# thimabru1010/ResUnet-a_mltsk_keras

Hardware: AMD Instinct MI355X
Metric: training patches/sec (256×256, 6-ch, bs=8/GPU) at 1/2/4/8 MI355X (higher is better)
Workload: dtype bf16; 1 GPU; cfg3: ResUnet-a d6 multitask (seg+bound+dist+color) Tanimoto-dual, 256x256x6, 6 classes, Adam, full train step (fwd+loss+bwd+allreduce+update); global_batch=8, per_gpu_batch=8, parallelism=dp1

## Files before the change

### include/rua_hip.h

```cpp
#ifndef RUA_HIP_H
#define RUA_HIP_H
#include <stdint.h>
#ifdef __cplusplus
extern "C" {
#endif

#define RUA_F32 0
#define RUA_BF16 1
#define RUA_MAX_SEG 6
#define RUA_MAX_BRANCH 4
#define RUA_MAX_WGRAD_BATCH 32
#define RUA_MAX_WGRAD_GROUP 8

#define RUA_OK 0
#define RUA_ERR_ARG (-1)
#define RUA_ERR_LAUNCH (-2)

int rua_version(void);
const char* rua_last_error(void);
int rua_device_info(int* cu_count, int* lds_bytes, char* arch, int arch_len);

typedef struct rua_conv_seg {
  const void* x;
  const void* w;
// ... 215 lines not shown
int rua_pixel_loss(int kind, const float* p, const float* z, const float* y, const float* class_w,
                   int64_t M, int C, double* loss_out, float* per_pixel, void* stream);
int rua_head_dz(int kind, int act, const float* p, const float* y, const float* coef, const float* class_w,
                float grad_scale, int B, int64_t HW, int C, float* dz, void* stream);
int rua_seg_metrics(const float* p, const float* y, int64_t M, int C, double* out, void* stream);

int rua_lr_step(double* state, float* lr_out, int adam, double beta1, double beta2, void* stream);
int rua_adam_step(float* theta, float* g, float* m, float* v, int64_t n, float lr_t, const float* lr_t_dev, float beta1, float beta2,
                  float eps, float grad_scale, int zero_grad, void* stream);
int rua_sgd_step(float* theta, float* g, float* vel, int64_t n, float lr, const float* lr_dev, float momentum, float grad_scale,
                 int zero_grad, void* stream);
int rua_adam_step_w(float* theta, float* g, float* m, float* v, int64_t n, float lr_t, const float* lr_t_dev, float beta1, float beta2,
                    float eps, float grad_scale, int zero_grad, void* wcopy_bf16, void* stream);
int rua_sgd_step_w(float* theta, float* g, float* vel, int64_t n, float lr, const float* lr_dev, float momentum, float grad_scale,
                   int zero_grad, void* wcopy_bf16, void* stream);

int64_t rua_targets_scratch_bytes(int N, int num_classes);
int rua_multitask_targets(const uint8_t* img, const uint8_t* cls, int N, int H, int W, int Cin, int num_classes, int norm_type,
                          float* x, float* seg, float* bound, float* dist, float* color, void* scratch, int64_t scratch_bytes, void* stream);

int rua_scene_windows(const uint8_t* const* scene_img, const uint8_t* const* scene_cls, const int32_t* scene_h, const int32_t* scene_w,
                      int nscenes, const int32_t* windows, int N, int PH, int PW, int Cin,
                      uint8_t* img_out, uint8_t* cls_out, void* stream);

int rua_scene_windows_affine(const uint8_t* const* scene_img, const uint8_t* const* scene_cls, const int32_t* scene_h, const int32_t* scene_w,
                             int nscenes, const int32_t* windows , int N, int PH, int PW, int Cin,
                             uint8_t* img_out, uint8_t* cls_out, void* stream);

int rua_scene_stitch(const float* p, int N, int PH, int PW, int C, const int32_t* windows, const int32_t* own,
                     uint8_t* const* scene_pred, const uint8_t* const* scene_cls, const int32_t* scene_h, const int32_t* scene_w,
// ... 32 lines not shown
```

### resunet_a_mltsk_keras_amd/_lib.py

```python
from __future__ import annotations

import ctypes as C
import os

HERE = os.path.dirname(os.path.abspath(__file__))
LIB_PATH = os.environ.get("RUA_LIB_PATH") or os.path.join(HERE, "librua_hip.so")

RUA_F32, RUA_BF16 = 0, 1
RUA_MAX_SEG, RUA_MAX_BRANCH, RUA_MAX_WGRAD_GROUP, RUA_MAX_WGRAD_BATCH = 6, 4, 8, 32
LOSS_TANIMOTO, LOSS_WCE, LOSS_CE_LOGITS, LOSS_BCE_LOGITS, LOSS_MSE = 0, 1, 2, 3, 4
ACT_NONE, ACT_SOFTMAX, ACT_SIGMOID = 0, 1, 2

vp, i32, i64, f32, f64 = C.c_void_p, C.c_int32, C.c_int64, C.c_float, C.c_double


class ConvSeg(C.Structure):
    _fields_ = [("x", vp), ("w", vp), ("C", i32), ("Hs", i32), ("Ws", i32), ("up_shift", i32), ("dil", i32), ("taps", i32)]


class ConvDesc(C.Structure):
    _fields_ = [("seg", ConvSeg * RUA_MAX_SEG), ("nseg", i32), ("N", i32), ("H", i32), ("W", i32), ("Cout", i32),
                ("stride", i32), ("dtype", i32), ("bias", vp), ("aux", vp), ("aux_mode", i32), ("mscale", vp),
                ("mshift", vp), ("out_relu", i32), ("accumulate", i32), ("y", vp), ("out_stride", i32), ("OH", i32),
                ("OW", i32), ("stats", vp), ("stats_mode", i32), ("workspace", vp), ("workspace_bytes", i64), ("stats_replicas", i32),
# ... 36 lines not shown


class BnBwdBranch(C.Structure):
    _fields_ = [("g", vp), ("stats2", vp), ("replicas", i32), ("stats2_out", i32), ("gamma", vp), ("mean", vp), ("rstd", vp),
                ("scale", vp), ("shift", vp), ("dgamma", vp), ("dbeta", vp)]


class BnBwdDesc(C.Structure):
    _fields_ = [("x", vp), ("dskip", vp), ("dx", vp), ("M", i64), ("C", i32), ("dtype", i32), ("nb", i32), ("masked", i32),
                ("accumulate", i32), ("pad", i32), ("count", f64), ("br", BnBwdBranch * RUA_MAX_BRANCH),
                ("skip_stats", vp), ("skip_replicas", i32), ("pad2", i32), ("dx_stats", vp), ("dx_replicas", i32), ("pad3", i32)]


class WprepItem(C.Structure):
    _fields_ = [("src_off", i64), ("dst_off", i64), ("taps", i32), ("Cout", i32), ("C", i32), ("pad", i32)]


PP = C.POINTER(vp)

_SIGS = {
    "rua_version": ([], i32),
    "rua_device_info": ([C.POINTER(i32), C.POINTER(i32), C.c_char_p, i32], i32),
    "rua_conv_fwd": ([C.POINTER(ConvDesc), vp], i32),
    "rua_conv_fwd_group": ([C.POINTER(ConvDesc), i32, vp], i32),
    "rua_conv_smem_bytes": ([C.POINTER(ConvDesc)], i32),
    "rua_conv_tile_bn": ([C.POINTER(ConvDesc)], i32),
    "rua_conv_tile_bm": ([C.POINTER(ConvDesc)], i32),
    "rua_conv_kernel_id": ([C.POINTER(ConvDesc)], i32),
    "rua_conv_fused_input_ok": ([C.POINTER(ConvDesc)], i32),
    "rua_conv_last_ksplit": ([], i32),
# ... 63 lines not shown
    "rua_fill_zero": ([vp, i64, vp], i32),
    "rua_tanimoto_sums": ([vp, vp, i32, i64, i32, vp, vp], i32),
    "rua_tanimoto_finalize": ([vp, i32, i64, i32, f32, vp, vp, vp, vp], i32),
    "rua_tanimoto_finalize_rep": ([vp, i32, i32, i64, i32, f32, vp, vp, vp, vp], i32),
    "rua_tanimoto_finalize_multi": ([vp, i32, vp], i32),
    "rua_head_dz_multi": ([vp, i32, vp], i32),
    "rua_tanimoto_ratio": ([vp, i32, i32, vp, vp, vp], i32),
    "rua_pixel_loss": ([i32, vp, vp, vp, vp, i64, i32, vp, vp, vp], i32),
    "rua_head_dz": ([i32, i32, vp, vp, vp, vp, f32, i32, i64, i32, vp, vp], i32),
    "rua_seg_metrics": ([vp, vp, i64, i32, vp, vp], i32),
    "rua_lr_step": ([vp, vp, i32, f64, f64, vp], i32),
    "rua_adam_step": ([vp, vp, vp, vp, i64, f32, vp, f32, f32, f32, f32, i32, vp], i32),
    "rua_sgd_step": ([vp, vp, vp, i64, f32, vp, f32, f32, i32, vp], i32),
    "rua_adam_step_w": ([vp, vp, vp, vp, i64, f32, vp, f32, f32, f32, f32, i32, vp, vp], i32),
    "rua_sgd_step_w": ([vp, vp, vp, i64, f32, vp, f32, f32, i32, vp, vp], i32),
    "rua_targets_scratch_bytes": ([i32, i32], i64),
    "rua_multitask_targets": ([vp, vp, i32, i32, i32, i32, i32, i32, vp, vp, vp, vp, vp, vp, i64, vp], i32),
    "rua_scene_windows": ([vp, vp, vp, vp, i32, vp, i32, i32, i32, i32, vp, vp, vp], i32),
    "rua_scene_windows_affine": ([vp, vp, vp, vp, i32, vp, i32, i32, i32, i32, vp, vp, vp], i32),
    "rua_scene_stitch": ([vp, i32, i32, i32, i32, vp, vp, vp, vp, vp, vp, i32, vp, vp], i32),
    "rua_scene_stitch_views": ([vp, i32, i32, i32, i32, i32, vp, vp, vp, vp, vp, vp, i32, vp, vp], i32),
    "rua_scene_stitch_maps": ([vp, i32, i32, i32, i32, i32, vp, vp, vp, vp, vp, i32, i32, vp], i32),
    "rua_scene_class_counts": ([vp, vp, vp, i32, vp, i32, i32, i32, i32, vp, vp], i32),
    "rua_scene_erode": ([vp, vp, vp, i32, i32, vp, vp, i32, vp, vp], i32),
    "rua_scene_boundary": ([vp, vp, vp, vp, i32, i32, i32, vp, vp, vp, vp], i32),
    "rua_set_tuning": ([C.c_char_p, i64], i32),
    "rua_get_tuning": ([C.c_char_p, C.POINTER(i64)], i32),
    "rua_tuning_key": ([i32], C.c_char_p),
}

# ... 66 lines not shown
```

### resunet_a_mltsk_keras_amd/build.py

```python
import os
import subprocess
import sys

HERE = os.path.dirname(os.path.abspath(__file__))
CSRC = os.path.join(HERE, "csrc")
OUT = os.environ.get("RUA_BUILD_OUT") or os.path.join(HERE, "librua_hip.so")
SOURCES = ["conv_mfma.hip", "conv_strip.hip", "conv_band.hip", "conv_band64.hip", "conv_band128.hip", "conv_img2.hip", "elementwise.hip", "small_conv.hip", "loss_optim.hip", "targets.hip", "scene.hip", "capi.cpp"]
FILE_FLAGS = {"conv_strip.hip": ["-fno-slp-vectorize"]}


def needs_build():
    if not os.path.exists(OUT):
        return True
    t = os.path.getmtime(OUT)
    deps = [os.path.join(CSRC, f) for f in os.listdir(CSRC)] + [os.path.join(HERE, "..", "include", "rua_hip.h")]
    return any(os.path.getmtime(d) > t for d in deps)


def build(force=False, verbose=True):
    if not force and not needs_build():
        return OUT
    hipcc = os.environ.get("HIPCC", "/opt/rocm/bin/hipcc")
    if not os.path.exists(hipcc):
        raise RuntimeError(f"hipcc not found at {hipcc}")
# ... 23 lines not shown
```

### resunet_a_mltsk_keras_amd/csrc/conv_mfma.hip

```cpp
#include "common.h"


template <typename T> __device__ __forceinline__ void load8(const unsigned char* base, size_t elem_off, float* f) {
  if constexpr (sizeof(T) == 2) {
    ET<T>::unpack(ldg16(base + elem_off * 2), f);
  } else {
    ET<T>::unpack(ldg16(base + elem_off * 4), f);
    ET<T>::unpack(ldg16(base + elem_off * 4 + 16), f + 4);
  }
}
template <typename T> __device__ __forceinline__ void store8(unsigned char* base, size_t elem_off, const float* f) {
  if constexpr (sizeof(T) == 2) {
    stg16(base + elem_off * 2, ET<T>::pack(f));
  } else {
    stg16(base + elem_off * 4, ET<T>::pack(f));
    stg16(base + elem_off * 4 + 16, ET<T>::pack(f + 4));
  }
}

template <typename T, int BM, int BN> __host__ __device__ constexpr int conv_smem_base() {
  constexpr int ROWB = (sizeof(T) == 2) ? 80 : 132;
  constexpr int a = 2 * (BM + BN) * ROWB;
  constexpr int b = BM * (BN + 4) * 4 + 4 * (BN / 8) * 16 * 4;
  return ((a > b ? a : b) + 15) / 16 * 16;
// ... 2295 lines not shown
}
struct WgKB { WgK k[RUA_MAX_WGRAD_BATCH]; unsigned end[RUA_MAX_WGRAD_BATCH]; int n; };
static_assert(sizeof(WgKB) <= 4096, "batched launch: kernel arguments are limited to 4 KiB");
__global__ __launch_bounds__(256) void wgrad_kernel_b(const WgKB g) {
  const unsigned b = blockIdx.x;
  int m = 0;
  for (int i = 0; i + 1 < g.n; ++i) m += (b >= g.end[i]) ? 1 : 0;
  const unsigned first = m ? g.end[m - 1] : 0u;
  wgrad_kernel_body<bf16_t>(g.k[m], (int)(b - first));
}

constexpr int SLAB_RED_COLS = 256;
__device__ __forceinline__ void wgrad_slab_reduce_body(const float* __restrict__ slabs, float* __restrict__ dw, long long n4, int ksplit, int vblock, int overwrite = 0) {
  const long long i = (long long)vblock * SLAB_RED_COLS + threadIdx.x;
  if (i >= n4) return;
  const float4* s = reinterpret_cast<const float4*>(slabs) + i;
  float4 t = make_float4(0.f, 0.f, 0.f, 0.f);
  auto add4 = [](float4& a, const float4 b) { a.x += b.x; a.y += b.y; a.z += b.z; a.w += b.w; };
  int k = 0;
  for (; k + 8 <= ksplit; k += 8) {
    float4 v[8];
#pragma unroll
    for (int u = 0; u < 8; ++u) v[u] = s[(size_t)(k + u) * n4];
    float4 a = v[0], b = v[4];
    add4(a, v[1]); add4(b, v[5]); add4(a, v[2]); add4(b, v[6]); add4(a, v[3]); add4(b, v[7]);
    add4(a, b); add4(t, a);
  }
  for (; k < ksplit; ++k) add4(t, s[(size_t)k * n4]);
  float4* d = reinterpret_cast<float4*>(dw) + i;
  float4 o = make_float4(0.f, 0.f, 0.f, 0.f);
  if (!overwrite) o = *d;
  add4(o, t);
  *d = o;
}
__global__ __launch_bounds__(256) void wgrad_slab_reduce(const float* __restrict__ slabs, float* __restrict__ dw, long long n4, int ksplit) {
  wgrad_slab_reduce_body(slabs, dw, n4, ksplit, (int)blockIdx.x);
}
static int launch_slab_reduce(const float* slabs, float* dw, long long n, int ksplit, hipStream_t st) {
  const long long n4 = n / 4;
  hipLaunchKernelGGL(wgrad_slab_reduce, dim3((unsigned)((n4 + SLAB_RED_COLS - 1) / SLAB_RED_COLS)), dim3(256), 0, st, slabs, dw, n4, ksplit);
  RUA_LAUNCH_CHECK("wgrad_slab_reduce");
  return RUA_OK;
}
static int slab_capacity(const rua_wgrad_desc* d, long long ndw);

struct WgdK {
  const unsigned char* a; const unsigned char* dy; float* dw;
  int C, Cout, H, W, dil, taps, wsh;
// ... 1199 lines not shown
#pragma unroll
    for (int q = 1; q < 4; ++q) v += *reinterpret_cast<const f32x4*>(src + q * 9 * 16 * 64);
    float* dst = p.dw + ((size_t)tap * p.Cout + co0 + col) * p.C + ci0 + c4;
    if (!ow) v += *reinterpret_cast<const f32x4*>(dst);
    *reinterpret_cast<f32x4*>(dst) = v;
  }
}

constexpr int TAPS_RED_COLS = 64;
__device__ __forceinline__ void wgrad_taps_reduce_body(const float* __restrict__ scratch, float* __restrict__ dw, int CC, int gx, int vblock, int overwrite = 0) {
  __shared__ float4 sh[256];
  const int total4 = 9 * CC * CC / 4;
  const int el = threadIdx.x & 63, sl = threadIdx.x >> 6;
  const int e4 = vblock * TAPS_RED_COLS + el;
  float4 s = make_float4(0.f, 0.f, 0.f, 0.f);
  auto add4 = [](float4& a, const float4 b) { a.x += b.x; a.y += b.y; a.z += b.z; a.w += b.w; };
  if (e4 < total4) {
    const int e = e4 * 4;
    const int tap = e / (CC * CC), r = e - tap * CC * CC, co = r / CC, ci = r - co * CC;
    const float* src = scratch + ((size_t)(co >> 5) * gx * 9 + tap) * 32 * CC + (co & 31) * CC + ci;
    const size_t pstride = (size_t)9 * 32 * CC;
    int b = sl;
    for (; b + 28 < gx; b += 32) {
      float4 v[8];
#pragma unroll
      for (int u = 0; u < 8; ++u) v[u] = *reinterpret_cast<const float4*>(src + (size_t)(b + 4 * u) * pstride);
      float4 a = v[0], c = v[4];
      add4(a, v[1]); add4(c, v[5]); add4(a, v[2]); add4(c, v[6]); add4(a, v[3]); add4(c, v[7]);
      add4(a, c); add4(s, a);
    }
    for (; b < gx; b += 4) add4(s, *reinterpret_cast<const float4*>(src + (size_t)b * pstride));
  }
  sh[threadIdx.x] = s;
  __syncthreads();
  if (sl == 0 && e4 < total4) {
    float4 t = sh[el];
    add4(t, sh[64 + el]); add4(t, sh[128 + el]); add4(t, sh[192 + el]);
    float4* d = reinterpret_cast<float4*>(dw + (size_t)e4 * 4);
    float4 o = make_float4(0.f, 0.f, 0.f, 0.f);
    if (!overwrite) o = *d;
    add4(o, t);
    *d = o;
  }
}

__global__ __launch_bounds__(256) void wgrad_taps_reduce(const float* __restrict__ scratch, float* __restrict__ dw, int CC, int gx) {
  wgrad_taps_reduce_body(scratch, dw, CC, gx, (int)blockIdx.x);
}

struct WgGroupCapture {
  int n;
  int kind[RUA_MAX_WGRAD_GROUP];
  unsigned gx[RUA_MAX_WGRAD_GROUP]; int smem[RUA_MAX_WGRAD_GROUP];
  WgK g[RUA_MAX_WGRAD_GROUP]; WgdK d[RUA_MAX_WGRAD_GROUP]; WgtK t[RUA_MAX_WGRAD_GROUP];
  int post[RUA_MAX_WGRAD_GROUP];
  const float* part[RUA_MAX_WGRAD_GROUP]; float* dw[RUA_MAX_WGRAD_GROUP]; long long ndw[RUA_MAX_WGRAD_GROUP]; int parts[RUA_MAX_WGRAD_GROUP], CC[RUA_MAX_WGRAD_GROUP], rblocks[RUA_MAX_WGRAD_GROUP];
};
// ... 1164 lines not shown
```

### resunet_a_mltsk_keras_amd/engine.py

```python
from __future__ import annotations

import ctypes as C
import math
import os
from dataclasses import dataclass, field
from typing import Dict, List, Optional, Tuple

import numpy as np
import torch

from . import _lib as L
from .scenes import MAP_HEADS, AffineSceneBatch, SceneBatch, check_radius, check_tolerance, check_views, view_rows

BN_EPS, BN_MOMENTUM, KERAS_EPS = 1e-3, 0.99, 1e-7
HEADS = ["seg", "bound", "dist", "color"]
SUMS_REPLICAS = 1


@dataclass
class ModelConfig:
    input_shape: Tuple[int, int, int] = (256, 256, 3)
    num_classes: int = 5
    multitasking: bool = False
    variant: str = "model2"
    width: int = 32
    depth: int = 6
# ... 249 lines not shown
        self.B = batch
        self.training = training
        self.dev = eng.dev
        self.dt = eng.dt
        self.tdt = torch.bfloat16 if eng.dt == L.RUA_BF16 else torch.float32
        self.vec = 8 if eng.dt == L.RUA_BF16 else 4
        self.fwd = Plan(dry)
        self.bwd = Plan(dry)
        self.loss_plan = Plan(dry)
        self.back_steps: List = _BackSteps(self)
        self.cur_tag: Optional[str] = None
        self.block_tag = ""
        self.pending: List[tuple] = []
        self.pending_bytes = 0
        self.pending_bucket = 0
        self.later: List[tuple] = []
        self.allocs: List[torch.Tensor] = []
        self.stats_used = 16
        self.act_bytes = 0
        self.img_u8 = self.cls_u8 = self.tgt_scratch = None
        self._build()

    def compact_buffers(self):
        if self.img_u8 is None:
            H, W, Cin = self.cfg.input_shape
            self.img_u8 = torch.empty((self.B, H, W, Cin), dtype=torch.uint8, device=self.dev)
            self.cls_u8 = torch.empty((self.B, H, W), dtype=torch.uint8, device=self.dev)
            n = int(L.lib().raw("rua_targets_scratch_bytes")(self.B, self.cfg.num_classes))
            self.tgt_scratch = torch.empty((max(n, 4),), dtype=torch.uint8, device=self.dev)
        return self.img_u8, self.cls_u8, self.tgt_scratch
# ... 408 lines not shown
        self.pending_bytes += nbytes

    def flush_wgrad(self, plan: Plan):
        self._issue_later(plan)
        self.pending_bytes = 0
        if not self.pending:
            return
        blocks = 0
        for r, _ in self.pending:
            r.block_begin = blocks
            blocks += r.blocks
        recs = (L.WgradPending * len(self.pending))(*[r for r, _ in self.pending])
        table = torch.frombuffer(bytearray(bytes(recs)), dtype=torch.uint8).to(self.dev)
        self.allocs.append(table)
        plan.add("rua_wgrad_reduce_batch", table.data_ptr(), len(self.pending), blocks, grads=[off for _, off in self.pending])
        self.pending = []

    def bias_grad(self, plan: Plan, dy: Ten, bias_offs: List[int]):
        s = self.col_stats(plan, dy)
        self.stats_to_grads(plan, s, dy.C, bias_offs)

    def stats_to_grads(self, plan: Plan, s: Stat, Cc: int, offs: List[int]):
        if self.dry or not (self.e.defer_reduce and plan is self.bwd):
            dst = L.ptr_array([self.G(o) for o in offs])
            plan.keep.append(dst)
            plan.add("rua_stats_to_f32", s.ptr, s.R, Cc, dst, len(offs), grads=offs)
            return
        for o in offs:
            bucket = self.e.dist.bucket_of(o) if self.e.dist is not None else 0
            if (self.pending or self.later) and bucket != self.pending_bucket:
                self.flush_wgrad(plan)
# ... 789 lines not shown
            raise L.RuaError("no HIP device visible: the ResUnet-a training path runs on MI355X only (there is no CPU fallback)")
        self.dev = device or torch.device("cuda", torch.cuda.current_device())
        cu = C.c_int32(0)
        if L.lib().raw("rua_device_info")(C.byref(cu), None, None, 0) == 0 and cu.value > 0:
            self.cu_count = cu.value
        z = lambda n, dt=torch.float32: torch.zeros(max(n, 16), dtype=dt, device=self.dev)
        self.P, self.G, self.M1, self.V1, self.S = z(ps.n), z(ps.n + ps.ns + 16), z(ps.n), z(ps.n), z(ps.ns)
        tdt = torch.bfloat16 if dtype == "bf16" else torch.float32
        self.Wf, self.Wd = z(ps.n, tdt), z(ps.n, tdt)
        self.wgrad_overwrite = os.environ.get("RUA_WGRAD_OVERWRITE", "1") != "0"
        self.ow_flag = torch.zeros(4, dtype=torch.int32, device=self.dev)
        self._ow = 0
        self._g_pending = False
        self.opt_wcopy = dtype == "bf16" and os.environ.get("RUA_OPT_WCOPY", "1") != "0"
        self.wf_fresh = False
        items = np.zeros(0, dtype=[("src", "<i8"), ("dst", "<i8"), ("taps", "<i4"), ("cout", "<i4"), ("c", "<i4"), ("pad", "<i4")])
        rows, mx = [], 1
        for lay in self.layers:
            if "segs" in lay and lay["mfma"]:
                for sg in lay["segs"]:
                    rows.append((sg["off"], sg["dst"], lay["taps"], lay["cout"], sg["C"], 0))
                    mx = max(mx, lay["taps"] * lay["cout"] * sg["C"])
        items = np.array(rows, dtype=items.dtype)
        self.wprep_items = torch.from_numpy(np.frombuffer(items.tobytes(), dtype=np.uint8).copy()).to(self.dev)
        self.wprep_n, self.wprep_max = len(rows), mx
        bm = []
        for i, (_, _, taps, cout, ci, _) in enumerate(rows):
            for b in range(L.lib().raw("rua_wprep_blocks")(taps, cout, ci)):
                bm += [i, 8 * b]
        self.wprep_map = torch.tensor(bm if bm else [0, 0], dtype=torch.int32, device=self.dev)
        self.wprep_map_n = len(bm) // 2
        self.stats_arena = torch.zeros(1 << 22, dtype=torch.float64, device=self.dev)
        self.workspace = torch.zeros(8 << 20, dtype=torch.float32, device=self.dev)
        self.scratch = torch.zeros(32 << 20, dtype=torch.float32, device=self.dev)
        self.lr_dev = torch.zeros(16, dtype=torch.float32, device=self.dev)
        self.lr_state = torch.zeros(2, dtype=torch.float64, device=self.dev)
        self._t_dev, self._lr_base_dev = -1, None
        self._dp_fence = torch.zeros(16, dtype=torch.float32, device=self.dev)
        self.use_graph = os.environ.get("RUA_USE_GRAPH", "1") != "0"
        self.group_1x1 = os.environ.get("RUA_GROUP_1X1", "1") != "0"
        self.group_heads = os.environ.get("RUA_GROUP_HEADS", "1") != "0"
        self.multi_head = os.environ.get("RUA_MULTI_HEAD", "1") != "0"
        self.merge_wgrad = {int(v) for v in os.environ.get("RUA_MERGE_WGRAD", "1,32,64,128,256").split(",") if v}
        self.group_wgrad_pw = os.environ.get("RUA_GROUP_WGRAD_PW", "1") != "0"
        self.batch_wgrad = os.environ.get("RUA_BATCH_WGRAD", "1") != "0"
        self.stem_mfma = os.environ.get("RUA_STEM_MFMA", "1") != "0"
# ... 57 lines not shown
        self._eval_seen = set()
        self._opt_graph = None
        self.graphs = {}
        cu = C.c_int32(0)
        if self.dev is not None and L.lib().raw("rua_device_info")(C.byref(cu), None, None, 0) == 0 and cu.value > 0:
            self.cu_count = cu.value

    def set_weights(self, keras_dict: Dict[str, np.ndarray]):
        P, S = self.params.from_keras(keras_dict)
        self.P.copy_(torch.from_numpy(P)); self.S.copy_(torch.from_numpy(S))
        self.params_changed()

    def params_changed(self):
        self.weights_dirty = True
        self.wf_fresh = False

    def get_weights(self) -> Dict[str, np.ndarray]:
        return self.params.to_keras(self.P.cpu().numpy(), self.S.cpu().numpy())

    def grads_keras(self) -> Dict[str, np.ndarray]:
        return self.params.to_keras(self.G.cpu().numpy())

    def count_params(self) -> int:
        return self.params.count()

    def _stream(self) -> int:
        return torch.cuda.current_stream(self.dev).cuda_stream

    def _prep_weights(self, s):
        if self.weights_dirty:
            if self.opt_wcopy and self.wf_fresh:
                L.lib().call("rua_weight_prep_dgrad", self.Wf.data_ptr(), self.Wd.data_ptr(), self.wprep_items.data_ptr(), self.wprep_n, self.wprep_max,
                             self.wprep_map.data_ptr() if self.wprep_map_n else None, self.wprep_map_n, self.dt, C.c_void_p(s))
            else:
                L.lib().call("rua_weight_prep", self.P.data_ptr(), self.Wf.data_ptr(), self.Wd.data_ptr(), self.wprep_items.data_ptr(),
                             self.wprep_n, self.wprep_max, self.dt, C.c_void_p(s))
                self.wf_fresh = True
            self.weights_dirty = False

    def _ensure_forward_copy(self):
        if self.opt_wcopy and not self.wf_fresh:
            self.weights_dirty = True
            self._prep_weights(self._stream())

    def _upload(self, g: Graph, x, y):
        def put(dst: torch.Tensor, src):
            if src is None:
                return
            if isinstance(src, np.ndarray):
                src = torch.from_numpy(np.ascontiguousarray(src, dtype=np.float32))
            if tuple(src.shape) != tuple(dst.shape):
                raise ValueError(f"expected shape {tuple(dst.shape)}, got {tuple(src.shape)}")
            dst.copy_(src, non_blocking=bool(src.is_pinned()) if isinstance(src, torch.Tensor) else False)
        put(g.x_in.t, x)
        if y is not None:
            if isinstance(y, dict):
# ... 129 lines not shown

    def _bucket_hooks(self, g: Graph):
        if getattr(g, "_hooks", None) is None:
            red = self.dist.reducer
            g._hooks = {idx: (lambda bs=bs: [red.ready(b) for b in bs]) for idx, bs in self._bucket_marks(g).items()}
        return g._hooks

    def _set_lr(self):
        sp = self.loss
        if self._t_dev != self.t or self._lr_base_dev != sp.lr:
            self.lr_state.copy_(torch.tensor([float(self.t), float(sp.lr)], dtype=torch.float64))
            self._t_dev, self._lr_base_dev = self.t, sp.lr
        self.t += 1
        self._t_dev += 1

    def _launch_optimizer(self, grad_scale, s):
        sp = self.loss
        L.lib().call("rua_lr_step", self.lr_state.data_ptr(), self.lr_dev.data_ptr(), 1 if sp.optimizer == "adam" else 0,
                     float(sp.beta_1), float(sp.beta_2), C.c_void_p(s))
        wc = self.Wf.data_ptr() if self.opt_wcopy else None
        if sp.optimizer == "adam":
            L.lib().call("rua_adam_step_w", self.P.data_ptr(), self.G.data_ptr(), self.M1.data_ptr(), self.V1.data_ptr(), self.params.n,
                         0.0, self.lr_dev.data_ptr(), sp.beta_1, sp.beta_2, KERAS_EPS, grad_scale, 1, wc, C.c_void_p(s))
        else:
            L.lib().call("rua_sgd_step_w", self.P.data_ptr(), self.G.data_ptr(), self.M1.data_ptr(), self.params.n, 0.0,
                         self.lr_dev.data_ptr(), sp.momentum, grad_scale, 1, wc, C.c_void_p(s))

    def optimizer_step(self, grad_scale: float = 1.0):
        self._set_lr()
        self._launch_optimizer(grad_scale, self._stream())
        self.weights_dirty = True
        self._g_pending = False

    def _issue_step(self, g: Graph):
        s = self._stream()
        self._zero_arena(g, s)
        self.weights_dirty = True
        self._prep_weights(s)
        g.fwd.run(s)
        g.loss_plan.run(s)
        g.bwd.run(s)
        self._launch_optimizer(1.0, s)

    def _graph_step(self, x, y, norm_type: Optional[int] = None):
        B = x.shape[0] if x is not None else self._last_B
        self._last_B = B
        g = self.graph(B, True)
        self._put_batch(g, x, y, norm_type)
        self._set_lr()
        self._set_overwrite(1 if (self.wgrad_overwrite and not self._g_pending) else 0)
        self._g_pending = False
        cap = self._captured.get(B)
        if cap is None:
            self._issue_step(g)
            torch.cuda.synchronize()
            cap = torch.cuda.CUDAGraph()
            with torch.cuda.graph(cap):
                self._issue_step(g)
            self._captured[B] = cap
            self.weights_dirty = True
            return g
        self._ensure_forward_copy()
        cap.replay()
        self.weights_dirty = True
        return g

    def count_step_dispatches(self, batch: int) -> Optional[int]:
        try:
            g = self.graph(batch, True)
            torch.cuda.synchronize()
            cap = torch.cuda.CUDAGraph(keep_graph=True)
            dirty, fresh = self.weights_dirty, self.wf_fresh
            with torch.cuda.graph(cap):
                self._issue_step(g)
            self.weights_dirty, self.wf_fresh = dirty, fresh
            k = C.c_int32(0)
            L.lib().call("rua_graph_kernel_nodes", C.c_void_p(cap.raw_cuda_graph()), C.byref(k), None)
            del cap
            return int(k.value)
        except Exception:
            torch.cuda.synchronize()
            return None

    def _graph_step_dp(self, x, y, norm_type: Optional[int] = None):
        B = x.shape[0] if x is not None else self._last_B
        self._last_B = B
        g = self.graph(B, True)
        self._put_batch(g, x, y, norm_type)
        red = self.dist.reducer
        pieces = self._captured_dp.get(B)
# ... 215 lines not shown
```

Before: 1343 patches/s.

## Fuse final wgrad reduction, optimizer update and bf16 weight-copy prep into one kernel

```diff
diff --git a/include/rua_hip.h b/include/rua_hip.h
--- a/include/rua_hip.h
+++ b/include/rua_hip.h
@@ -253,6 +253,19 @@
                     float eps, float grad_scale, int zero_grad, void* wcopy_bf16, void* stream);
 int rua_sgd_step_w(float* theta, float* g, float* vel, int64_t n, float lr, const float* lr_dev, float momentum, float grad_scale,
                    int zero_grad, void* wcopy_bf16, void* stream);
+typedef struct rua_optim_fused {
+  int32_t optimizer, pad;
+  float* theta; float* g; float* m; float* v;
+  int64_t n;
+  float lr; const float* lr_dev;
+  float beta1, beta2, eps, momentum, grad_scale, pad2;
+  void* w_fwd; void* w_dgrad;
+  const rua_wprep_item* items; int32_t n_items, n_pending;
+  const int32_t* item_rec;
+  const rua_wgrad_pending* pending;
+  const int32_t* blockmap; int32_t n_blocks, pad3;
+} rua_optim_fused;
+int rua_optim_step_fused(const rua_optim_fused* d, void* stream);
 
 int64_t rua_targets_scratch_bytes(int N, int num_classes);
 int rua_multitask_targets(const uint8_t* img, const uint8_t* cls, int N, int H, int W, int Cin, int num_classes, int norm_type,
diff --git a/resunet_a_mltsk_keras_amd/_lib.py b/resunet_a_mltsk_keras_amd/_lib.py
--- a/resunet_a_mltsk_keras_amd/_lib.py
+++ b/resunet_a_mltsk_keras_amd/_lib.py
@@ -74,6 +74,12 @@
 
 class WprepItem(C.Structure):
     _fields_ = [("src_off", i64), ("dst_off", i64), ("taps", i32), ("Cout", i32), ("C", i32), ("pad", i32)]
+
+
+class OptimFused(C.Structure):
+    _fields_ = [("optimizer", i32), ("pad", i32), ("theta", vp), ("g", vp), ("m", vp), ("v", vp), ("n", i64), ("lr", f32), ("lr_dev", vp),
+                ("beta1", f32), ("beta2", f32), ("eps", f32), ("momentum", f32), ("grad_scale", f32), ("pad2", f32), ("w_fwd", vp), ("w_dgrad", vp),
+                ("items", vp), ("n_items", i32), ("n_pending", i32), ("item_rec", vp), ("pending", vp), ("blockmap", vp), ("n_blocks", i32), ("pad3", i32)]
 
 
 PP = C.POINTER(vp)
@@ -167,6 +173,7 @@
     "rua_sgd_step": ([vp, vp, vp, i64, f32, vp, f32, f32, i32, vp], i32),
     "rua_adam_step_w": ([vp, vp, vp, vp, i64, f32, vp, f32, f32, f32, f32, i32, vp, vp], i32),
     "rua_sgd_step_w": ([vp, vp, vp, i64, f32, vp, f32, f32, i32, vp, vp], i32),
+    "rua_optim_step_fused": ([C.POINTER(OptimFused), vp], i32),
     "rua_targets_scratch_bytes": ([i32, i32], i64),
     "rua_multitask_targets": ([vp, vp, i32, i32, i32, i32, i32, i32, vp, vp, vp, vp, vp, vp, i64, vp], i32),
     "rua_scene_windows": ([vp, vp, vp, vp, i32, vp, i32, i32, i32, i32, vp, vp, vp], i32),
diff --git a/resunet_a_mltsk_keras_amd/build.py b/resunet_a_mltsk_keras_amd/build.py
--- a/resunet_a_mltsk_keras_amd/build.py
+++ b/resunet_a_mltsk_keras_amd/build.py
@@ -5,7 +5,7 @@
 HERE = os.path.dirname(os.path.abspath(__file__))
 CSRC = os.path.join(HERE, "csrc")
 OUT = os.environ.get("RUA_BUILD_OUT") or os.path.join(HERE, "librua_hip.so")
-SOURCES = ["conv_mfma.hip", "conv_strip.hip", "conv_band.hip", "conv_band64.hip", "conv_band128.hip", "conv_img2.hip", "elementwise.hip", "small_conv.hip", "loss_optim.hip", "targets.hip", "scene.hip", "capi.cpp"]
+SOURCES = ["conv_mfma.hip", "conv_strip.hip", "conv_band.hip", "conv_band64.hip", "conv_band128.hip", "conv_img2.hip", "elementwise.hip", "small_conv.hip", "loss_optim.hip", "optim_fused.hip", "targets.hip", "scene.hip", "capi.cpp"]
 FILE_FLAGS = {"conv_strip.hip": ["-fno-slp-vectorize"]}
 
 
diff --git a/resunet_a_mltsk_keras_amd/csrc/conv_mfma.hip b/resunet_a_mltsk_keras_amd/csrc/conv_mfma.hip
--- a/resunet_a_mltsk_keras_amd/csrc/conv_mfma.hip
+++ b/resunet_a_mltsk_keras_amd/csrc/conv_mfma.hip
@@ -1,4 +1,5 @@
 #include "common.h"
+#include "wgrad_reduce.h"
 
 
 template <typename T> __device__ __forceinline__ void load8(const unsigned char* base, size_t elem_off, float* f) {
@@ -2333,24 +2334,11 @@
 __device__ __forceinline__ void wgrad_slab_reduce_body(const float* __restrict__ slabs, float* __restrict__ dw, long long n4, int ksplit, int vblock, int overwrite = 0) {
   const long long i = (long long)vblock * SLAB_RED_COLS + threadIdx.x;
   if (i >= n4) return;
-  const float4* s = reinterpret_cast<const float4*>(slabs) + i;
-  float4 t = make_float4(0.f, 0.f, 0.f, 0.f);
-  auto add4 = [](float4& a, const float4 b) { a.x += b.x; a.y += b.y; a.z += b.z; a.w += b.w; };
-  int k = 0;
-  for (; k + 8 <= ksplit; k += 8) {
-    float4 v[8];
-#pragma unroll
-    for (int u = 0; u < 8; ++u) v[u] = s[(size_t)(k + u) * n4];
-    float4 a = v[0], b = v[4];
-    add4(a, v[1]); add4(b, v[5]); add4(a, v[2]); add4(b, v[6]); add4(a, v[3]); add4(b, v[7]);
-    add4(a, b); add4(t, a);
-  }
-  for (; k < ksplit; ++k) add4(t, s[(size_t)k * n4]);
+  const float4 t = wgrad_slab_sum(reinterpret_cast<const float4*>(slabs) + i, (size_t)n4, ksplit);
   float4* d = reinterpret_cast<float4*>(dw) + i;
   float4 o = make_float4(0.f, 0.f, 0.f, 0.f);
   if (!overwrite) o = *d;
-  add4(o, t);
-  *d = o;
+  *d = wgrad_finish(o, t);
 }
 __global__ __launch_bounds__(256) void wgrad_slab_reduce(const float* __restrict__ slabs, float* __restrict__ dw, long long n4, int ksplit) {
   wgrad_slab_reduce_body(slabs, dw, n4, ksplit, (int)blockIdx.x);
@@ -3580,33 +3568,15 @@
   const int el = threadIdx.x & 63, sl = threadIdx.x >> 6;
   const int e4 = vblock * TAPS_RED_COLS + el;
   float4 s = make_float4(0.f, 0.f, 0.f, 0.f);
-  auto add4 = [](float4& a, const float4 b) { a.x += b.x; a.y += b.y; a.z += b.z; a.w += b.w; };
-  if (e4 < total4) {
-    const int e = e4 * 4;
-    const int tap = e / (CC * CC), r = e - tap * CC * CC, co = r / CC, ci = r - co * CC;
-    const float* src = scratch + ((size_t)(co >> 5) * gx * 9 + tap) * 32 * CC + (co & 31) * CC + ci;
-    const size_t pstride = (size_t)9 * 32 * CC;
-    int b = sl;
-    for (; b + 28 < gx; b += 32) {
-      float4 v[8];
-#pragma unroll
-      for (int u = 0; u < 8; ++u) v[u] = *reinterpret_cast<const float4*>(src + (size_t)(b + 4 * u) * pstride);
-      float4 a = v[0], c = v[4];
-      add4(a, v[1]); add4(c, v[5]); add4(a, v[2]); add4(c, v[6]); add4(a, v[3]); add4(c, v[7]);
-      add4(a, c); add4(s, a);
-    }
-    for (; b < gx; b += 4) add4(s, *reinterpret_cast<const float4*>(src + (size_t)b * pstride));
-  }
+  if (e4 < total4) s = wgrad_taps_lane_sum(wgrad_taps_src(scratch, CC, gx, e4 * 4), wgrad_taps_pstride(CC), gx, sl);
   sh[threadIdx.x] = s;
   __syncthreads();
   if (sl == 0 && e4 < total4) {
-    float4 t = sh[el];
-    add4(t, sh[64 + el]); add4(t, sh[128 + el]); add4(t, sh[192 + el]);
+    const float4 t = wgrad_taps_fold(sh[el], sh[64 + el], sh[128 + el], sh[192 + el]);
     float4* d = reinterpret_cast<float4*>(dw + (size_t)e4 * 4);
     float4 o = make_float4(0.f, 0.f, 0.f, 0.f);
     if (!overwrite) o = *d;
-    add4(o, t);
-    *d = o;
+    *d = wgrad_finish(o, t);
   }
 }
 
diff --git a/resunet_a_mltsk_keras_amd/csrc/optim_fused.hip b/resunet_a_mltsk_keras_amd/csrc/optim_fused.hip
--- /dev/null
+++ b/resunet_a_mltsk_keras_amd/csrc/optim_fused.hip
@@ -0,0 +1,236 @@
+#include "common.h"
+#include "wgrad_reduce.h"
+
+struct AdamUpd {
+  static constexpr bool HAS_V = true;
+  float lr, b1, b2, eps, gs;
+  template <bool TAIL>
+  __device__ __forceinline__ void apply(float gg_, float& mm, float& vv, float& tt) const {
+#pragma clang fp contract(off)
+    const float gg = gg_ * gs, a1 = 1.f - b1, a2 = 1.f - b2;
+    if constexpr (TAIL) { mm = __builtin_fmaf(b1, mm, a1 * gg); vv = __builtin_fmaf(b2, vv, (a2 * gg) * gg); }
+    else { mm = __builtin_fmaf(a1, gg, b1 * mm); vv = __builtin_fmaf(gg, a2 * gg, b2 * vv); }
+    const float q = (lr * mm) / (sqrtf(vv) + eps);
+    tt = tt - q;
+  }
+};
+struct SgdUpd {
+  static constexpr bool HAS_V = false;
+  float lr, mu, gs;
+  template <bool TAIL>
+  __device__ __forceinline__ void apply(float gg, float& vel, float&, float& tt) const {
+#pragma clang fp contract(off)
+    const float vv = __builtin_fmaf(mu, vel, -((lr * gg) * gs));
+    vel = vv;
+    tt = tt + vv;
+  }
+};
+
+struct OptK {
+  float* th; float* g; float* m; float* v;
+  unsigned short* wf; unsigned short* wd;
+  const rua_wprep_item* items; const int* item_rec; const rua_wgrad_pending* pend; const int4* blockmap; const float* lr_dev;
+  long long ntail;
+};
+
+__device__ __forceinline__ float4 ld4(const float* p) { return *reinterpret_cast<const float4*>(p); }
+__device__ __forceinline__ void st4(float* p, const float4 v) { *reinterpret_cast<float4*>(p) = v; }
+
+template <typename U>
+__device__ __forceinline__ uint2 update4(const OptK& k, const U& u, size_t i, const float4 g4) {
+  float4 m4 = ld4(k.m + i), t4 = ld4(k.th + i), v4 = make_float4(0.f, 0.f, 0.f, 0.f);
+  if constexpr (U::HAS_V) v4 = ld4(k.v + i);
+  u.template apply<false>(g4.x, m4.x, v4.x, t4.x); u.template apply<false>(g4.y, m4.y, v4.y, t4.y); u.template apply<false>(g4.z, m4.z, v4.z, t4.z); u.template apply<false>(g4.w, m4.w, v4.w, t4.w);
+  st4(k.m + i, m4); st4(k.th + i, t4);
+  if constexpr (U::HAS_V) st4(k.v + i, v4);
+  return make_uint2(ET<bf16_t>::pk(t4.x, t4.y), ET<bf16_t>::pk(t4.z, t4.w));
+}
+template <typename U>
+__device__ __forceinline__ unsigned short update1(const OptK& k, const U& u, size_t i, float gg) {
+  float mm = k.m[i], tt = k.th[i], vv = 0.f;
+  if constexpr (U::HAS_V) vv = k.v[i];
+  if ((long long)i >= k.ntail) u.template apply<true>(gg, mm, vv, tt); else u.template apply<false>(gg, mm, vv, tt);
+  k.m[i] = mm; k.th[i] = tt;
+  if constexpr (U::HAS_V) k.v[i] = vv;
+  return __builtin_bit_cast(unsigned short, (bf16_t)tt);
+}
+
+template <int RK>
+__device__ __forceinline__ float4 grad4(float* __restrict__ garena, const float* __restrict__ part, int parts, int CC, size_t n_item, int e, bool ow) {
+  const float4 zero = make_float4(0.f, 0.f, 0.f, 0.f);
+  if constexpr (RK == 0) {
+    const float4 g4 = ld4(garena + e);
+    st4(garena + e, zero);
+    return g4;
+  } else {
+    float4 t;
+    if constexpr (RK == 1) {
+      const float* src = wgrad_taps_src(part, CC, parts, e);
+      const size_t ps = wgrad_taps_pstride(CC);
+      const float4 s0 = wgrad_taps_lane_sum(src, ps, parts, 0); __builtin_amdgcn_sched_barrier(0);
+      const float4 s1 = wgrad_taps_lane_sum(src, ps, parts, 1); __builtin_amdgcn_sched_barrier(0);
+      const float4 s2 = wgrad_taps_lane_sum(src, ps, parts, 2); __builtin_amdgcn_sched_barrier(0);
+      const float4 s3 = wgrad_taps_lane_sum(src, ps, parts, 3); __builtin_amdgcn_sched_barrier(0);
+      t = wgrad_taps_fold(s0, s1, s2, s3);
+    } else {
+      t = wgrad_slab_sum(reinterpret_cast<const float4*>(part + e), n_item / 4, parts);
+    }
+    float4 o = zero;
+    if (!ow) { o = ld4(garena + e); st4(garena + e, zero); }
+    return wgrad_finish(o, t);
+  }
+}
+
+template <typename U, int RK>
+__device__ __forceinline__ void tile_rows(const OptK& k, const U& u, const rua_wprep_item& it, int t, int tco, int tci, const float* part, int parts, int CC, bool ow) {
+  const int lane = threadIdx.x & 63, cg = lane >> 3, pg = lane & 7;
+  const int tap = t / (tco * tci), r = t - tap * tco * tci;
+  const int co = (r / tci) * 64 + cg * 8, ci = (r % tci) * 64 + pg * 8;
+  if (co >= it.Cout || ci >= it.C) return;
+  const size_t n_item = (size_t)it.taps * it.Cout * it.C;
+  uint4 in[8];
+#pragma unroll
+  for (int q = 0; q < 8; ++q) in[q] = make_uint4(0u, 0u, 0u, 0u);
+#pragma nounroll
+  for (int j = 0; j < 8; ++j) {
+    const int e = (tap * it.Cout + co + j) * it.C + ci;
+    const float4 g0 = grad4<RK>(k.g + it.src_off, part, parts, CC, n_item, e, ow);
+    if constexpr (RK != 0) __builtin_amdgcn_sched_barrier(0);
+    const float4 g1 = grad4<RK>(k.g + it.src_off, part, parts, CC, n_item, e + 4, ow);
+    const uint2 lo = update4(k, u, (size_t)it.src_off + e, g0), hi = update4(k, u, (size_t)it.src_off + e + 4, g1);
+    const uint4 pk = make_uint4(lo.x, lo.y, hi.x, hi.y);
+    *reinterpret_cast<uint4*>(k.wf + it.dst_off + e) = pk;
+#pragma unroll
+    for (int q = 0; q < 8; ++q) if (q == j) in[q] = pk;
+  }
+  unsigned short* dp = k.wd + it.dst_off + (size_t)(it.taps - 1 - tap) * it.Cout * it.C + (size_t)ci * it.Cout + co;
+#pragma unroll
+  for (int i = 0; i < 8; ++i) {
+    unsigned e[8];
+#pragma unroll
+    for (int j = 0; j < 8; ++j) {
+      const unsigned w = (i >> 1) == 0 ? in[j].x : (i >> 1) == 1 ? in[j].y : (i >> 1) == 2 ? in[j].z : in[j].w;
+      e[j] = (i & 1) ? (w >> 16) : (w & 0xffffu);
+    }
+    *reinterpret_cast<uint4*>(dp + (size_t)i * it.Cout) = make_uint4(e[0] | (e[1] << 16), e[2] | (e[3] << 16), e[4] | (e[5] << 16), e[6] | (e[7] << 16));
+  }
+}
+
+template <typename U>
+__global__ __launch_bounds__(256) void optim_fused_kernel(const OptK k, U u) {
+  __shared__ unsigned short tile[64][66];
+  if (k.lr_dev) u.lr = k.lr_dev[0];
+  const int4 bm = k.blockmap[blockIdx.x];
+  const int tid = threadIdx.x;
+  if (bm.x == 0) {
+#pragma unroll
+    for (int q = 0; q < 4; ++q) {
+      const int c = q * 256 + tid;
+      if (c < bm.w) {
+        const size_t i = ((size_t)bm.z + c) * 4;
+        const float4 g4 = ld4(k.g + i);
+        st4(k.g + i, make_float4(0.f, 0.f, 0.f, 0.f));
+        *reinterpret_cast<uint2*>(k.wf + i) = update4(k, u, i, g4);
+      }
+    }
+    return;
+  }
+  if (bm.x == 3) {
+    if (tid < bm.w) {
+      const size_t i = (size_t)bm.z + tid;
+      const float gg = k.g[i];
+      k.g[i] = 0.f;
+      k.wf[i] = update1(k, u, i, gg);
+    }
+    return;
+  }
+  const rua_wprep_item it = k.items[bm.y];
+  const int rec = k.item_rec ? k.item_rec[bm.y] : -1;
+  int rk = 0, parts = 0, CC = 0; const float* part = nullptr; bool ow = false;
+  if (rec >= 0) {
+    const rua_wgrad_pending p = k.pend[rec];
+    rk = p.kind; parts = p.parts; CC = p.CC; part = p.partials;
+    ow = p.overwrite_dev && *p.overwrite_dev != 0;
+  }
+  const int tco = (it.Cout + 63) / 64, tci = (it.C + 63) / 64;
+  if (bm.x == 1) {
+    const int wv = tid >> 6;
+    for (int t = bm.z + wv; t < bm.z + bm.w; t += 4) {
+      if (rk == 1) tile_rows<U, 1>(k, u, it, t, tco, tci, part, parts, CC, ow);
+      else if (rk == 2) tile_rows<U, 2>(k, u, it, t, tco, tci, part, parts, CC, ow);
+      else tile_rows<U, 0>(k, u, it, t, tco, tci, part, parts, CC, ow);
+    }
+    return;
+  }
+  const int tx = tid & 15, ty = tid >> 4;
+  const size_t n_item = (size_t)it.taps * it.Cout * it.C;
+  const bool vec = (it.C % 4 == 0) && (it.Cout % 4 == 0);
+  for (int t = bm.z; t < bm.z + bm.w; ++t) {
+    const int tap = t / (tco * tci), r = t - tap * tco * tci;
+    const int co0 = (r / tci) * 64, ci0 = (r % tci) * 64;
+#pragma nounroll
+    for (int q = 0; q < 4; ++q) {
+      const int co = co0 + ty + q * 16;
+#pragma nounroll
+      for (int j = 0; j < 4; ++j) {
+        const int ci = ci0 + tx * 4 + j;
+        unsigned short b = 0;
+        if (co < it.Cout && ci < it.C) {
+          const size_t e = (size_t)tap * it.Cout * it.C + (size_t)co * it.C + ci, i = (size_t)it.src_off + e;
+          float gg;
+          if (rk == 2) {
+            const float s = wgrad_slab_sum(part + e, n_item, parts);
+            float o = 0.f;
+            if (!ow) { o = k.g[i]; k.g[i] = 0.f; }
+            gg = wgrad_finish(o, s);
+          } else { gg = k.g[i]; k.g[i] = 0.f; }
+          b = update1(k, u, i, gg);
+          k.wf[it.dst_off + e] = b;
+        }
+        tile[ty + q * 16][tx * 4 + j] = b;
+      }
+    }
+    __syncthreads();
+#pragma unroll
+    for (int q = 0; q < 4; ++q) {
+      const int ci = ci0 + ty + q * 16, co = co0 + tx * 4;
+      if (ci < it.C) {
+        unsigned short v[4];
+#pragma unroll
+        for (int j = 0; j < 4; ++j) v[j] = tile[tx * 4 + j][ty + q * 16];
+        unsigned short* d = k.wd + it.dst_off + (size_t)(it.taps - 1 - tap) * it.Cout * it.C + (size_t)ci * it.Cout + co;
+        if (vec && co + 3 < it.Cout) *reinterpret_cast<uint2*>(d) = make_uint2((unsigned)v[0] | ((unsigned)v[1] << 16), (unsigned)v[2] | ((unsigned)v[3] << 16));
+        else {
+#pragma unroll
+          for (int j = 0; j < 4; ++j) if (co + j < it.Cout) d[j] = v[j];
+        }
+      }
+    }
+    __syncthreads();
+  }
+}
+
+extern "C" int rua_optim_step_fused(const rua_optim_fused* d, void* stream) {
+  RUA_CHECK_ARG(d, "rua_optim_step_fused: null descriptor");
+  RUA_CHECK_ARG(d->theta && d->g && d->m && (d->v || d->optimizer == 1) && d->n > 0 && d->n < ((int64_t)1 << 31), "rua_optim_step_fused: bad buffers");
+  RUA_CHECK_ARG(d->optimizer == 0 || d->optimizer == 1, "rua_optim_step_fused: optimizer must be 0 (Adam) or 1 (SGD)");
+  RUA_CHECK_ARG(d->w_fwd && d->w_dgrad && d->w_fwd != d->w_dgrad, "rua_optim_step_fused: needs both bf16 weight copies");
+  RUA_CHECK_ARG((((size_t)d->theta | (size_t)d->g | (size_t)d->m | (size_t)d->v | (size_t)d->w_fwd | (size_t)d->w_dgrad) & 15) == 0, "rua_optim_step_fused: buffers must be 16-byte aligned");
+  RUA_CHECK_ARG(d->blockmap && d->n_blocks >= 1 && ((size_t)d->blockmap & 15) == 0, "rua_optim_step_fused: needs a block map (16-byte aligned)");
+  RUA_CHECK_ARG(d->n_items >= 0 && (d->n_items == 0 || d->items), "rua_optim_step_fused: bad item table");
+  RUA_CHECK_ARG(d->n_pending >= 0 && (d->n_pending == 0 || (d->pending && d->item_rec)), "rua_optim_step_fused: pending records need their table and the items' record indices");
+  OptK k;
+  k.th = d->theta; k.g = d->g; k.m = d->m; k.v = d->v;
+  k.wf = (unsigned short*)d->w_fwd; k.wd = (unsigned short*)d->w_dgrad;
+  k.items = d->items; k.item_rec = d->n_pending > 0 ? d->item_rec : nullptr; k.pend = d->pending;
+  k.blockmap = (const int4*)d->blockmap; k.lr_dev = d->lr_dev; k.ntail = d->n & ~(int64_t)3;
+  if (d->optimizer == 0) {
+    const AdamUpd u{d->lr, d->beta1, d->beta2, d->eps, d->grad_scale};
+    hipLaunchKernelGGL((optim_fused_kernel<AdamUpd>), dim3(d->n_blocks), dim3(256), 0, (hipStream_t)stream, k, u);
+  } else {
+    const SgdUpd u{d->lr, d->momentum, d->grad_scale};
+    hipLaunchKernelGGL((optim_fused_kernel<SgdUpd>), dim3(d->n_blocks), dim3(256), 0, (hipStream_t)stream, k, u);
+  }
+  RUA_LAUNCH_CHECK("rua_optim_step_fused");
+  return RUA_OK;
+}
diff --git a/resunet_a_mltsk_keras_amd/csrc/wgrad_reduce.h b/resunet_a_mltsk_keras_amd/csrc/wgrad_reduce.h
--- /dev/null
+++ b/resunet_a_mltsk_keras_amd/csrc/wgrad_reduce.h
@@ -0,0 +1,50 @@
+#pragma once
+#include <hip/hip_runtime.h>
+
+__device__ __forceinline__ void rua_acc(float4& a, const float4 b) { a.x += b.x; a.y += b.y; a.z += b.z; a.w += b.w; }
+__device__ __forceinline__ void rua_acc(float& a, const float b) { a += b; }
+template <typename V> __device__ __forceinline__ V rua_vzero();
+template <> __device__ __forceinline__ float4 rua_vzero<float4>() { return make_float4(0.f, 0.f, 0.f, 0.f); }
+template <> __device__ __forceinline__ float rua_vzero<float>() { return 0.f; }
+
+template <typename V>
+__device__ __forceinline__ V wgrad_slab_sum(const V* __restrict__ s, size_t stride, int ksplit) {
+  V t = rua_vzero<V>();
+  int k = 0;
+  for (; k + 8 <= ksplit; k += 8) {
+    V v[8];
+#pragma unroll
+    for (int u = 0; u < 8; ++u) v[u] = s[(size_t)(k + u) * stride];
+    V a = v[0], b = v[4];
+    rua_acc(a, v[1]); rua_acc(b, v[5]); rua_acc(a, v[2]); rua_acc(b, v[6]); rua_acc(a, v[3]); rua_acc(b, v[7]);
+    rua_acc(a, b); rua_acc(t, a);
+  }
+  for (; k < ksplit; ++k) rua_acc(t, s[(size_t)k * stride]);
+  return t;
+}
+
+__device__ __forceinline__ size_t wgrad_taps_pstride(int CC) { return (size_t)9 * 32 * CC; }
+__device__ __forceinline__ const float* wgrad_taps_src(const float* __restrict__ scratch, int CC, int gx, int e) {
+  const int tap = e / (CC * CC), r = e - tap * CC * CC, co = r / CC, ci = r - co * CC;
+  return scratch + ((size_t)(co >> 5) * gx * 9 + tap) * 32 * CC + (co & 31) * CC + ci;
+}
+__device__ __forceinline__ float4 wgrad_taps_lane_sum(const float* __restrict__ src, size_t pstride, int gx, int sl) {
+  float4 s = make_float4(0.f, 0.f, 0.f, 0.f);
+  int b = sl;
+  for (; b + 28 < gx; b += 32) {
+    float4 v[8];
+#pragma unroll
+    for (int u = 0; u < 8; ++u) v[u] = *reinterpret_cast<const float4*>(src + (size_t)(b + 4 * u) * pstride);
+    float4 a = v[0], c = v[4];
+    rua_acc(a, v[1]); rua_acc(c, v[5]); rua_acc(a, v[2]); rua_acc(c, v[6]); rua_acc(a, v[3]); rua_acc(c, v[7]);
+    rua_acc(a, c); rua_acc(s, a);
+  }
+  for (; b < gx; b += 4) rua_acc(s, *reinterpret_cast<const float4*>(src + (size_t)b * pstride));
+  return s;
+}
+__device__ __forceinline__ float4 wgrad_taps_fold(float4 s0, const float4 s1, const float4 s2, const float4 s3) {
+  rua_acc(s0, s1); rua_acc(s0, s2); rua_acc(s0, s3);
+  return s0;
+}
+template <typename V>
+__device__ __forceinline__ V wgrad_finish(V old, const V t) { rua_acc(old, t); return old; }
diff --git a/resunet_a_mltsk_keras_amd/engine.py b/resunet_a_mltsk_keras_amd/engine.py
--- a/resunet_a_mltsk_keras_amd/engine.py
+++ b/resunet_a_mltsk_keras_amd/engine.py
@@ -10,6 +10,7 @@
 import torch
 
 from . import _lib as L
+from . import optim_map
 from .scenes import MAP_HEADS, AffineSceneBatch, SceneBatch, check_radius, check_tolerance, check_views, view_rows
 
 BN_EPS, BN_MOMENTUM, KERAS_EPS = 1e-3, 0.99, 1e-7
@@ -289,6 +290,8 @@
         self.pending: List[tuple] = []
         self.pending_bytes = 0
         self.pending_bucket = 0
+        self.last_flush = None
+        self._tail = None
         self.later: List[tuple] = []
         self.allocs: List[torch.Tensor] = []
         self.stats_used = 16
@@ -727,7 +730,32 @@
         table = torch.frombuffer(bytearray(bytes(recs)), dtype=torch.uint8).to(self.dev)
         self.allocs.append(table)
         plan.add("rua_wgrad_reduce_batch", table.data_ptr(), len(self.pending), blocks, grads=[off for _, off in self.pending])
+        self.last_flush = (len(plan.calls) - 1, [r for r, _ in self.pending])
         self.pending = []
+
+    def optim_tail(self) -> Optional[dict]:
+        if self._tail is None and self.last_flush is not None and self.last_flush[0] == len(self.bwd.calls) - 1:
+            e = self.e
+            recs = self.last_flush[1]
+            fused, residual = optim_map.split_pending(recs, e.wprep_rows, e.G.data_ptr())
+            up = lambda arr: torch.frombuffer(bytearray(bytes(arr)), dtype=torch.uint8).to(self.dev)
+            t = dict(n_fused=len(fused), n_res=len(residual), res_blocks=0, fused_idx=fused, res_idx=residual)
+            if fused:
+                t["fused"] = up((L.WgradPending * len(fused))(*[recs[j] for _, j in fused]))
+                item_rec = np.full(max(len(e.wprep_rows), 1), -1, np.int32)
+                cost = [0] * len(e.wprep_rows)
+                for k, (i, j) in enumerate(fused):
+                    item_rec[i], cost[i] = k, recs[j].parts
+                t["item_rec"] = torch.from_numpy(item_rec).to(self.dev)
+                t["map"] = torch.from_numpy(optim_map.block_map(e.wprep_rows, e.params.n, cost)).to(self.dev)
+            if residual:
+                rr = [L.WgradPending.from_buffer_copy(recs[j]) for j in residual]
+                for r in rr:
+                    r.block_begin = t["res_blocks"]
+                    t["res_blocks"] += r.blocks
+                t["res"] = up((L.WgradPending * len(rr))(*rr))
+            self._tail = t
+        return self._tail
 
     def bias_grad(self, plan: Plan, dy: Ten, bias_offs: List[int]):
         s = self.col_stats(plan, dy)
@@ -1547,13 +1575,12 @@
         self._g_pending = False
         self.opt_wcopy = dtype == "bf16" and os.environ.get("RUA_OPT_WCOPY", "1") != "0"
         self.wf_fresh = False
+        self.fused_tail = self.opt_wcopy and os.environ.get("RUA_FUSED_TAIL", "1") != "0"
+        self.wd_fresh = False
         items = np.zeros(0, dtype=[("src", "<i8"), ("dst", "<i8"), ("taps", "<i4"), ("cout", "<i4"), ("c", "<i4"), ("pad", "<i4")])
-        rows, mx = [], 1
-        for lay in self.layers:
-            if "segs" in lay and lay["mfma"]:
-                for sg in lay["segs"]:
-                    rows.append((sg["off"], sg["dst"], lay["taps"], lay["cout"], sg["C"], 0))
-                    mx = max(mx, lay["taps"] * lay["cout"] * sg["C"])
+        rows = optim_map.conv_rows(self.layers)
+        mx = max([1] + [t * co * ci for _, _, t, co, ci, _ in rows])
+        self.wprep_rows = rows
         items = np.array(rows, dtype=items.dtype)
         self.wprep_items = torch.from_numpy(np.frombuffer(items.tobytes(), dtype=np.uint8).copy()).to(self.dev)
         self.wprep_n, self.wprep_max = len(rows), mx
@@ -1563,6 +1590,8 @@
                 bm += [i, 8 * b]
         self.wprep_map = torch.tensor(bm if bm else [0, 0], dtype=torch.int32, device=self.dev)
         self.wprep_map_n = len(bm) // 2
+        if self.fused_tail:
+            self.optim_map = torch.from_numpy(optim_map.block_map(rows, ps.n)).to(self.dev)
         self.stats_arena = torch.zeros(1 << 22, dtype=torch.float64, device=self.dev)
         self.workspace = torch.zeros(8 << 20, dtype=torch.float32, device=self.dev)
         self.scratch = torch.zeros(32 << 20, dtype=torch.float32, device=self.dev)
@@ -1650,6 +1679,7 @@
     def params_changed(self):
         self.weights_dirty = True
         self.wf_fresh = False
+        self.wd_fresh = False
 
     def get_weights(self) -> Dict[str, np.ndarray]:
         return self.params.to_keras(self.P.cpu().numpy(), self.S.cpu().numpy())
@@ -1665,17 +1695,20 @@
 
     def _prep_weights(self, s):
         if self.weights_dirty:
-            if self.opt_wcopy and self.wf_fresh:
+            if self.opt_wcopy and self.wf_fresh and self.wd_fresh:
+                pass
+            elif self.opt_wcopy and self.wf_fresh:
                 L.lib().call("rua_weight_prep_dgrad", self.Wf.data_ptr(), self.Wd.data_ptr(), self.wprep_items.data_ptr(), self.wprep_n, self.wprep_max,
                              self.wprep_map.data_ptr() if self.wprep_map_n else None, self.wprep_map_n, self.dt, C.c_void_p(s))
+                self.wd_fresh = True
             else:
                 L.lib().call("rua_weight_prep", self.P.data_ptr(), self.Wf.data_ptr(), self.Wd.data_ptr(), self.wprep_items.data_ptr(),
                              self.wprep_n, self.wprep_max, self.dt, C.c_void_p(s))
-                self.wf_fresh = True
+                self.wf_fresh = self.wd_fresh = True
             self.weights_dirty = False
 
     def _ensure_forward_copy(self):
-        if self.opt_wcopy and not self.wf_fresh:
+        if self.opt_wcopy and not (self.wf_fresh and (self.wd_fresh or not self.fused_tail)):
             self.weights_dirty = True
             self._prep_weights(self._stream())
 
@@ -1835,10 +1868,26 @@
         self.t += 1
         self._t_dev += 1
 
-    def _launch_optimizer(self, grad_scale, s):
+    def _launch_optimizer(self, grad_scale, s, tail=None):
         sp = self.loss
         L.lib().call("rua_lr_step", self.lr_state.data_ptr(), self.lr_dev.data_ptr(), 1 if sp.optimizer == "adam" else 0,
                      float(sp.beta_1), float(sp.beta_2), C.c_void_p(s))
+        if self.fused_tail:
+            d = L.OptimFused()
+            d.optimizer = 0 if sp.optimizer == "adam" else 1
+            d.theta, d.g, d.m, d.v, d.n = self.P.data_ptr(), self.G.data_ptr(), self.M1.data_ptr(), self.V1.data_ptr(), self.params.n
+            d.lr, d.lr_dev = 0.0, self.lr_dev.data_ptr()
+            d.beta1, d.beta2, d.eps, d.momentum, d.grad_scale = sp.beta_1, sp.beta_2, KERAS_EPS, sp.momentum, grad_scale
+            d.w_fwd, d.w_dgrad = self.Wf.data_ptr(), self.Wd.data_ptr()
+            d.items, d.n_items = self.wprep_items.data_ptr(), self.wprep_n
+            bm = self.optim_map
+            if tail is not None and tail["n_fused"]:
+                d.item_rec, d.pending, d.n_pending = tail["item_rec"].data_ptr(), tail["fused"].data_ptr(), tail["n_fused"]
+                bm = tail["map"]
+            d.blockmap, d.n_blocks = bm.data_ptr(), bm.shape[0]
+            L.lib().call("rua_optim_step_fused", C.byref(d), C.c_void_p(s))
+            return
+        self.wd_fresh = False
         wc = self.Wf.data_ptr() if self.opt_wcopy else None
         if sp.optimizer == "adam":
             L.lib().call("rua_adam_step_w", self.P.data_ptr(), self.G.data_ptr(), self.M1.data_ptr(), self.V1.data_ptr(), self.params.n,
@@ -1860,8 +1909,14 @@
         self._prep_weights(s)
         g.fwd.run(s)
         g.loss_plan.run(s)
-        g.bwd.run(s)
-        self._launch_optimizer(1.0, s)
+        tail = g.optim_tail() if self.fused_tail else None
+        if tail is None:
+            g.bwd.run(s)
+        else:
+            g.bwd.run(s, last=len(g.bwd.calls) - 1)
+            if tail["n_res"]:
+                L.lib().call("rua_wgrad_reduce_batch", tail["res"].data_ptr(), tail["n_res"], tail["res_blocks"], C.c_void_p(s))
+        self._launch_optimizer(1.0, s, tail)
 
     def _graph_step(self, x, y, norm_type: Optional[int] = None):
         B = x.shape[0] if x is not None else self._last_B
@@ -1891,10 +1946,12 @@
             g = self.graph(batch, True)
             torch.cuda.synchronize()
             cap = torch.cuda.CUDAGraph(keep_graph=True)
-            dirty, fresh = self.weights_dirty, self.wf_fresh
+            dirty, fresh, dfresh = self.weights_dirty, self.wf_fresh, self.wd_fresh
+            if self.fused_tail:
+                self.wf_fresh = self.wd_fresh = True
             with torch.cuda.graph(cap):
                 self._issue_step(g)
-            self.weights_dirty, self.wf_fresh = dirty, fresh
+            self.weights_dirty, self.wf_fresh, self.wd_fresh = dirty, fresh, dfresh
             k = C.c_int32(0)
             L.lib().call("rua_graph_kernel_nodes", C.c_void_p(cap.raw_cuda_graph()), C.byref(k), None)
             del cap
diff --git a/resunet_a_mltsk_keras_amd/optim_map.py b/resunet_a_mltsk_keras_amd/optim_map.py
--- /dev/null
+++ b/resunet_a_mltsk_keras_amd/optim_map.py
@@ -0,0 +1,114 @@
+from __future__ import annotations
+
+from typing import List, Optional, Sequence, Tuple
+
+import numpy as np
+
+K_FLAT, K_TILES, K_TILES_LDS, K_SCALAR = 0, 1, 2, 3
+FLAT4 = 1024
+TILES = 4
+SCALAR = 256
+
+
+def conv_rows(layers) -> List[tuple]:
+    rows = []
+    for lay in layers:
+        if "segs" in lay and lay["mfma"]:
+            for sg in lay["segs"]:
+                rows.append((sg["off"], sg["dst"], lay["taps"], lay["cout"], sg["C"], 0))
+    return rows
+
+
+def item_tiles(taps: int, cout: int, c: int) -> int:
+    return taps * ((cout + 63) // 64) * ((c + 63) // 64)
+
+
+def item_fast(cout: int, c: int) -> bool:
+    return c % 8 == 0 and cout % 8 == 0
+
+
+def _flat_blocks(a: int, b: int, out: list):
+    def scalar(lo, hi):
+        for f in range(lo, hi, SCALAR):
+            out.append((K_SCALAR, -1, f, min(SCALAR, hi - f)))
+    a4, b4 = (a + 3) // 4 * 4, b // 4 * 4
+    if a4 >= b4:
+        scalar(a, b)
+        return
+    scalar(a, a4)
+    for f in range(a4 // 4, b4 // 4, FLAT4):
+        out.append((K_FLAT, -1, f, min(FLAT4, b4 // 4 - f)))
+    scalar(b4, b)
+
+
+def block_map(rows: Sequence[tuple], n: int, item_cost: Optional[Sequence[int]] = None, tiles: int = TILES) -> np.ndarray:
+    order = sorted(range(len(rows)), key=lambda i: rows[i][0])
+    blocks: list = []
+    pos = 0
+    for i in order:
+        src, dst, taps, cout, c, _ = rows[i]
+        size = taps * cout * c
+        if src != dst:
+            raise ValueError(f"item {i}: the weight copies must share the master's index space (dst_off {dst} != src_off {src})")
+        if src < pos or src + size > n:
+            raise ValueError(f"item {i}: [{src}, {src + size}) overlaps its neighbour or leaves [0, {n})")
+        fast = item_fast(cout, c)
+        if fast and src % 8 != 0:
+            raise ValueError(f"item {i}: offset {src} is not 16-byte aligned in the bf16 copies")
+        if src > pos:
+            _flat_blocks(pos, src, blocks)
+        nt = item_tiles(taps, cout, c)
+        for t in range(0, nt, tiles):
+            blocks.append((K_TILES if fast else K_TILES_LDS, i, t, min(tiles, nt - t)))
+        pos = src + size
+    if pos < n:
+        _flat_blocks(pos, n, blocks)
+    if item_cost is not None:
+        blocks.sort(key=lambda b: -(item_cost[b[1]] if b[1] >= 0 else 0))
+    return np.asarray(blocks, dtype=np.int32).reshape(-1, 4)
+
+
+def coverage(bm: np.ndarray, rows: Sequence[tuple], n: int) -> np.ndarray:
+    cnt = np.zeros(n, np.int32)
+    for kind, item, first, count in bm.tolist():
+        if kind == K_FLAT:
+            cnt[first * 4:(first + count) * 4] += 1
+        elif kind == K_SCALAR:
+            cnt[first:first + count] += 1
+        else:
+            src, _, taps, cout, c, _ = rows[item]
+            tco, tci = (cout + 63) // 64, (c + 63) // 64
+            view = cnt[src:src + taps * cout * c].reshape(taps, cout, c)
+            for t in range(first, first + count):
+                tap, r = divmod(t, tco * tci)
+                co0, ci0 = (r // tci) * 64, (r % tci) * 64
+                view[tap, co0:co0 + 64, ci0:ci0 + 64] += 1
+    return cnt
+
+
+def split_pending(records: Sequence, rows: Sequence[tuple], g_ptr: int) -> Tuple[List[Tuple[int, int]], List[int]]:
+    by_off = {r[0]: i for i, r in enumerate(rows)}
+    cand: dict = {}
+    residual: List[int] = []
+    for j, r in enumerate(records):
+        item = None
+        if r.kind in (1, 2) and (r.dw - g_ptr) % 4 == 0:
+            i = by_off.get((r.dw - g_ptr) // 4)
+            if i is not None:
+                _, _, taps, cout, c, _ = rows[i]
+                if r.n == taps * cout * c and r.parts >= 1:
+                    if r.kind == 1 and taps == 9 and cout == c == r.CC and c in (32, 64):
+                        item = i
+                    elif r.kind == 2 and r.n % 4 == 0:
+                        item = i
+        if item is None:
+            residual.append(j)
+        else:
+            cand.setdefault(item, []).append(j)
+    fused = []
+    for item, js in cand.items():
+        if len(js) == 1:
+            fused.append((item, js[0]))
+        else:
+            residual += js
+    return sorted(fused), sorted(residual)
```

After: 1306 patches/s. -2.8%, worse.
